# reczoo/FuxiCTR

Measured on NVIDIA H100. Metric: samples/sec DeepFM Criteo-shape train_step (fwd+bwd+clip+Adam), higher is better.
Workload: dtype f32 (3xTF32 tensor-core GEMMs, fp32 everything else)

## Files before the change

fuxictr_b200/_lib.py:

```python
import ctypes
import os

HERE = os.path.dirname(os.path.abspath(__file__))
LIB_PATH = os.path.join(HERE, "libfuxictr_b200.so")

B2_F32, B2_BF16, B2_F64, B2_I64, B2_I32 = 0, 1, 2, 3, 4
B2_POOL_NONE, B2_POOL_SUM, B2_POOL_MEAN = 0, 1, 2
B2_ACT_NONE, B2_ACT_RELU, B2_ACT_SIGMOID = 0, 1, 2
B2_PREP_MUL = 3
B2_GEMM_C_IS_ZERO, B2_GEMM_COLSUM_IS_ZERO, B2_GEMM_X3_INLINE, B2_GEMM_BACKFILL = 1, 2, 4, 8
B2_MAX_FIELDS = 128
FM_PRODUCT_SUM, FM_BI_INTERACTION, FM_INNER_PRODUCT = 0, 1, 2

c_void_p, c_int, c_int32, c_int64, c_float = (ctypes.c_void_p, ctypes.c_int, ctypes.c_int32,
                                              ctypes.c_int64, ctypes.c_float)


class b2_lazy_ctx(ctypes.Structure):
    _fields_ = [
        ("last_step", ctypes.c_void_p), ("sched", ctypes.c_void_p), ("step_dev", ctypes.c_void_p),
        ("mark", ctypes.c_void_p), ("worklist", ctypes.c_void_p), ("counter", ctypes.c_void_p),
        ("delta_m", ctypes.c_int64), ("delta_v", ctypes.c_int64),
        ("w1", ctypes.c_float), ("beta2", ctypes.c_float), ("w2", ctypes.c_float), ("eps", ctypes.c_float),
        ("worklist_capacity", ctypes.c_int32), ("pad_", ctypes.c_int32),
        ("grow_emb", ctypes.c_int64 * 128), ("grow_lr", ctypes.c_int64 * 128),
    ]


class b2_lazy_table(ctypes.Structure):
    _fields_ = [("param", ctypes.c_void_p), ("rows", ctypes.c_int64), ("grow_base", ctypes.c_int64),
                ("dim", ctypes.c_int32), ("pad_", ctypes.c_int32)]


class b2_field(ctypes.Structure):
    _fields_ = [
        ("table", c_void_p), ("idx", c_void_p), ("out", c_void_p),
        ("vocab", c_int64), ("idx_stride", c_int64), ("out_stride", c_int64),
        ("dim", c_int32), ("seq_len", c_int32), ("pool", c_int32), ("padding_idx", c_int32),
    ]


class b2_touch(ctypes.Structure):
    _fields_ = [("flags", c_void_p), ("base", c_void_p), ("n", c_int64)]


_FIELD_P = ctypes.POINTER(b2_field)


class b2_gemm_desc(ctypes.Structure):
    _fields_ = [
        ("a", c_void_p), ("b", c_void_p), ("a_small", c_void_p), ("b_small", c_void_p),
        ("c", c_void_p), ("c_small", c_void_p), ("c_pre", c_void_p), ("bias", c_void_p), ("mul", c_void_p), ("add", c_void_p),
        ("ybwd", c_void_p), ("colsum", c_void_p),
        ("lda", c_int64), ("ldb", c_int64), ("ldc", c_int64), ("M", c_int64), ("N", c_int64), ("K", c_int64),
        ("a_mn_major", c_int32), ("b_mn_major", c_int32), ("act", c_int32), ("act_bwd", c_int32),
        ("beta_accumulate", c_int32), ("elem_dtype", c_int32), ("ld_aux", c_int64),
        ("flags", c_int64),
        ("drop_rng", c_void_p), ("drop_layer", c_int64), ("drop_thresh", ctypes.c_uint32), ("drop_scale", c_float),
    ]

class b2_gemm_plan(ctypes.Structure):
    _fields_ = [(k, c_int32) for k in ("bn", "splits", "stages", "cstages", "grid", "threads", "tiles_m", "tiles_n",
                                       "passes", "kb_per_split")] + \
               [("smem_bytes", c_int64)]


SIGNATURES = {
    "b2_version": (ctypes.c_char_p, []),
    "b2_last_error": (ctypes.c_char_p, []),
    "b2_device_cc": (c_int, [c_int]),
    "b2_set_l2_fetch_granularity": (c_int, [c_int]),
    "b2_embed_gather_fwd": (c_int, [_FIELD_P, c_int, c_int64, c_int, c_int, c_void_p, c_void_p, c_void_p]),
    "b2_embed_gather_hot_fwd": (c_int, [_FIELD_P, c_int, c_int64, c_int, c_int, c_void_p, c_void_p, c_int, c_void_p]),
    "b2_embed_scatter_bwd": (c_int, [_FIELD_P, c_int, c_int64, c_int, c_int, c_void_p, c_void_p]),
    "b2_embed_scatter_bwd_ex": (c_int, [_FIELD_P, c_int, c_int64, c_int, c_int, c_void_p, c_void_p, c_void_p]),
    "b2_lr_fwd": (c_int, [_FIELD_P, c_int, c_int64, c_int, c_void_p, c_void_p, c_void_p, c_void_p]),
    "b2_lr_bwd": (c_int, [_FIELD_P, c_int, c_int64, c_int, c_void_p, c_void_p, c_void_p]),
    "b2_lr_bwd_ex": (c_int, [_FIELD_P, c_int, c_int64, c_int, c_void_p, c_void_p, c_void_p, c_void_p]),
    "b2_front_fwd": (c_int, [_FIELD_P, _FIELD_P, c_int, c_int64, c_int, c_int, c_void_p, c_void_p, c_void_p,
                             c_void_p, c_void_p, c_void_p, c_void_p]),
    "b2_front_bwd": (c_int, [_FIELD_P, _FIELD_P, c_int, c_int64, c_int, c_int, c_void_p, c_void_p, c_void_p,
                             c_void_p, c_void_p, c_void_p, c_void_p]),
    "b2_front_bwd_ex": (c_int, [_FIELD_P, _FIELD_P, c_int, c_int64, c_int, c_int, c_void_p, c_void_p, c_void_p,
                                c_void_p, c_void_p, c_void_p, c_void_p, c_void_p]),
    "b2_lazy_sumsq": (c_int, [c_void_p, c_int, c_void_p, c_void_p, c_int, c_int64, c_void_p, c_void_p]),
    "b2_lazy_adam_step": (c_int, [c_void_p, c_int, c_void_p, c_void_p, c_int, c_int64, c_int64, c_int64, c_void_p,
                                  c_void_p, c_void_p, c_void_p, c_float, c_float, c_float, c_float, c_void_p]),
    "b2_lazy_materialize": (c_int, [c_void_p, c_int, c_int64, c_int64, c_int64, c_void_p, c_void_p, c_void_p,
                                    c_float, c_float, c_float, c_void_p]),
    "b2_adam_sched": (c_int, [c_void_p, c_float, c_float, c_float, c_void_p, c_int64, c_void_p]),
    "b2_adam_step_sched": (c_int, [c_void_p, c_void_p, c_void_p, c_void_p, c_int64, c_void_p, c_float, c_float,
                                   c_float, c_float, c_void_p, c_void_p, c_int, c_void_p]),
    "b2_shard_push": (c_int, [_FIELD_P, _FIELD_P, c_int, c_int64, c_int, c_int, c_void_p, c_int, c_int64,
                              c_void_p, c_void_p, c_void_p, c_void_p, c_void_p, c_int32, c_void_p]),
    "b2_shard_pull": (c_int, [_FIELD_P, _FIELD_P, c_int, c_int64, c_int, c_int, c_void_p, c_void_p, c_float,
                              c_void_p, c_void_p, c_int32, c_void_p]),
    "b2_shard_push_ex": (c_int, [_FIELD_P, _FIELD_P, c_int, c_int64, c_int, c_int, c_void_p, c_int, c_int64,
                                 c_void_p, c_void_p, c_void_p, c_void_p, c_void_p, c_int32, c_void_p, c_void_p]),
    "b2_shard_pull_ex": (c_int, [_FIELD_P, _FIELD_P, c_int, c_int64, c_int, c_int, c_void_p, c_void_p, c_float,
                                 c_void_p, c_void_p, c_int32, c_void_p, c_void_p, c_void_p]),
    "b2_shard_push_pad": (c_int, [_FIELD_P, _FIELD_P, c_int, c_int64, c_int, c_int, c_void_p, c_int, c_int64,
                                  c_void_p, c_void_p, c_void_p, c_void_p, c_void_p, c_int32, c_void_p, c_void_p,
                                  c_void_p]),
    "b2_shard_publish_ids": (c_int, [c_void_p, c_int, c_int64, c_void_p, _FIELD_P, _FIELD_P, c_int, c_int, c_int,
                                     c_void_p, c_void_p]),
    "b2_shard_publish_rows": (c_int, [c_void_p, c_int, c_int64, c_int64, c_int64, c_void_p, _FIELD_P, _FIELD_P, c_int,
                                      c_int, c_int, c_void_p, c_void_p, c_void_p]),
    "b2_shard_lookup": (c_int, [_FIELD_P, _FIELD_P, c_int, c_int64, c_int, c_int, c_void_p, c_int64, c_void_p, c_void_p,
                                c_void_p, c_void_p, c_void_p, c_void_p]),
    "b2_peer_bcast": (c_int, [c_void_p, c_int64, c_void_p, c_int, c_void_p]),
    "b2_peer_bcast_ids": (c_int, [c_void_p, c_int, c_int64, c_void_p, c_int, c_void_p]),
# ... 106 lines not shown
```

fuxictr_b200/csrc/gemm_tc.cu:

```cuda
#include "b2_common.cuh"
#include "philox.cuh"
#include <string.h>
#include <cstdlib>
#include <cuda.h>

namespace tc {
constexpr int BM = 128;
constexpr int NTHREADS = 384;
constexpr int NCONV = 96;
constexpr int BACKFILL_KB = 16;
enum Mode { TF32 = 0, BF16 = 1, X3 = 2 };

struct Ring {
  uint32_t off_b, off_as, off_bs, off_sa, off_sb;
  uint32_t stage;
  int stages;
  size_t smem;
};
constexpr uint32_t RING_EXTRA = 1024 + 128;
constexpr uint32_t SMEM_MAX = 227u * 1024u;
constexpr Ring ring_layout(int bn, int mode, bool a_mn, bool b_mn) {
  const uint32_t a = BM * 128, b = (uint32_t) bn * 128;
  Ring r{};
  uint32_t o = a;
// ... 5 lines not shown
  r.stage = o;
  r.stages = (SMEM_MAX - RING_EXTRA) / o >= 4 ? 4 : (int) ((SMEM_MAX - RING_EXTRA) / o);
  r.smem = (size_t) r.stages * o + RING_EXTRA;
  return r;
}
constexpr size_t ring_smem_max(int bn, int mode) {
  size_t m = 0;
  for (int a_mn = 0; a_mn < 2; ++a_mn)
    for (int b_mn = 0; b_mn < 2; ++b_mn) {
      const size_t s = ring_layout(bn, mode, a_mn != 0, b_mn != 0).smem;
      m = s > m ? s : m;
    }
  return m;
}
static_assert(ring_layout(128, TF32, true, true).stages >= 2 && ring_layout(64, X3, true, true).stages >= 2,
              "ring does not fit shared memory");
constexpr int epi_pitch(int bn) { return bn + 8; }
constexpr uint32_t epi_bytes(int bn) { return (uint32_t) (BM * epi_pitch(bn) + 256 * 4) * 4u; }
constexpr bool epi_fits(int bn, int mode) {
  for (int a_mn = 0; a_mn < 2; ++a_mn)
    for (int b_mn = 0; b_mn < 2; ++b_mn) {
      const Ring r = ring_layout(bn, mode, a_mn != 0, b_mn != 0);
      if ((uint32_t) r.stages * r.stage < epi_bytes(bn)) return false;
    }
  return true;
}
static_assert(epi_fits(32, TF32) && epi_fits(64, TF32) && epi_fits(128, TF32) && epi_fits(32, BF16) &&
              epi_fits(64, BF16) && epi_fits(128, BF16) && epi_fits(32, X3) && epi_fits(64, X3),
              "epilogue tile does not fit the ring");

struct Params {
  CUtensorMap map_a;
  CUtensorMap map_b;
  float* c;
  float* c_small;
  float* c_pre;
  int64_t ldc;
  const float* bias;
  const float* mul;
  const float* add;
  const float* ybwd;
  float* colsum;
  int M, N, K, act, act_bwd, beta, kb_per_split;
  int a_mn, b_mn;
  int esz;
  int64_t ld_aux;
  int vec;
  int tiles_m, tiles_n, splits;
  Ring ring;
  const int64_t* drop_rng;
  int64_t drop_layer;
  uint32_t drop_thresh;
  float drop_scale;
};

__device__ __forceinline__ uint32_t smem_u32(const void* p) {
  return (uint32_t) __cvta_generic_to_shared(p);
}
__device__ __forceinline__ void mbar_init(uint32_t bar, uint32_t count) {
  asm volatile("mbarrier.init.shared::cta.b64 [%0], %1;" ::"r"(bar), "r"(count) : "memory");
}
__device__ __forceinline__ void mbar_expect_tx(uint32_t bar, uint32_t bytes) {
  asm volatile("mbarrier.arrive.expect_tx.shared::cta.b64 _, [%0], %1;" ::"r"(bar), "r"(bytes)
               : "memory");
}
__device__ __forceinline__ void mbar_arrive(uint32_t bar) {
  asm volatile("mbarrier.arrive.shared::cta.b64 _, [%0];" ::"r"(bar) : "memory");
}
__device__ __forceinline__ bool mbar_try_wait(uint32_t bar, uint32_t parity) {
  uint32_t ok;
  asm volatile(
      "{\n"
      ".reg .pred p;\n"
      "mbarrier.try_wait.parity.shared::cta.b64 p, [%1], %2;\n"
      "selp.u32 %0, 1, 0, p;\n"
      "}\n"
      : "=r"(ok)
      : "r"(bar), "r"(parity)
      : "memory");
  return ok != 0;
}
__device__ __forceinline__ void mbar_wait(uint32_t bar, uint32_t parity) {
  if (mbar_try_wait(bar, parity)) return;
  const long long t0 = clock64();
  while (!mbar_try_wait(bar, parity))
    if (clock64() - t0 > 4000000000LL) __trap();
}
__device__ __forceinline__ void tma_load_2d(uint32_t dst, const CUtensorMap* map, uint32_t bar,
                                            int c0, int c1) {
  asm volatile(
      "cp.async.bulk.tensor.2d.shared::cluster.global.mbarrier::complete_tx::bytes [%0], [%1, {%2, %3}], [%4];"
      ::"r"(dst), "l"(reinterpret_cast<uint64_t>(map)), "r"(c0), "r"(c1), "r"(bar)
      : "memory");
}
__device__ __forceinline__ uint64_t make_smem_desc(uint32_t addr) {
  uint64_t d = 0;
  d |= (uint64_t) ((addr & 0x3FFFFu) >> 4);
  d |= (uint64_t) 1 << 16;
  d |= (uint64_t) (1024 >> 4) << 32;
  d |= (uint64_t) 1 << 62;
  return d;
}
__device__ __forceinline__ uint32_t swz(int r, int c) { return (uint32_t) (r * 128 + ((c ^ (r & 7)) << 4)); }
__device__ __forceinline__ float tf32_small(float v) { return b2_tf32_small(v); }
__device__ __forceinline__ float tf32_big(float v) { return __uint_as_float(__float_as_uint(v) & 0xffffe000u); }
__device__ __forceinline__ void wgmma_fence() { asm volatile("wgmma.fence.sync.aligned;" ::: "memory"); }
// ... 361 lines not shown
    constexpr int SEG = BM * SPR / 256;
    constexpr int BATCH = 4;
    const int et = threadIdx.x - 128;
    const int c4 = et % SPR, r0 = et / SPR;
    const int n = n0 + 4 * c4;
    const int nv = min(4, p.N - n);
    const bool vec_n = p.vec && nv == 4;
    const float4 bv = (p.bias != nullptr && z == 0 && nv > 0) ? seg_load<true>(p.bias + n, vec_n, nv)
                                                             : make_float4(0.f, 0.f, 0.f, 0.f);
    float cs[4] = {0.f, 0.f, 0.f, 0.f};
    uint64_t dseed = 0, doff = 0;
    if constexpr (DROP) {
      dseed = (uint64_t) p.drop_rng[0];
      doff = (uint64_t) p.drop_rng[1] + (uint64_t) p.drop_layer;
    }
#pragma unroll 1
    for (int b0 = 0; b0 < SEG; b0 += BATCH) {
      float4 mv[BATCH], av[BATCH], yv[BATCH], cv[BATCH];
#pragma unroll
      for (int i = 0; i < BATCH; ++i) {
        const int m = m0 + r0 + (256 / SPR) * (b0 + i);
        const int k = m < p.M ? nv : 0;
        const bool v = vec_n && m < p.M;
        const int64_t o = (int64_t) m * p.ldc + n;
        const float4 zero = make_float4(0.f, 0.f, 0.f, 0.f);
        mv[i] = p.mul != nullptr ? seg_load<true>(p.mul + o, v, k) : zero;
        av[i] = p.add != nullptr ? seg_load<true>(p.add + o, v, k) : zero;
        yv[i] = p.ybwd != nullptr ? seg_load<true>(p.ybwd + o, v, k) : zero;
        cv[i] = (p.beta && p.splits == 1) ? seg_load<false>(p.c + o, v, k) : zero;
      }
#pragma unroll
      for (int i = 0; i < BATCH; ++i) {
        const int r = r0 + (256 / SPR) * (b0 + i);
        const int m = m0 + r;
        const int k = m < p.M ? nv : 0;
        const bool v = vec_n && m < p.M;
        const int64_t o = (int64_t) m * p.ldc + n;
        const float4 a = *reinterpret_cast<const float4*>(tile + r * P + 4 * c4);
        float4 t = make_float4(__fadd_rn(a.x, bv.x), __fadd_rn(a.y, bv.y), __fadd_rn(a.z, bv.z), __fadd_rn(a.w, bv.w));
        if (p.splits > 1) {
          seg_red_add(p.c + o, t, v, k);
          continue;
        }
        if (p.c_pre != nullptr) seg_store(p.c_pre + o, t, v, k);
        uint32_t kb = 0;
        if constexpr (DROP) {
          if (k > 0) kb = b2_drop_keep4(dseed, doff, (uint64_t) m * (uint64_t) p.N + (uint64_t) n, k, p.drop_thresh);
        }
        t.x = epilogue_elem<DROP>(p, t.x, mv[i].x, av[i].x, yv[i].x, cv[i].x, kb & 1u);
        t.y = epilogue_elem<DROP>(p, t.y, mv[i].y, av[i].y, yv[i].y, cv[i].y, kb & 2u);
        t.z = epilogue_elem<DROP>(p, t.z, mv[i].z, av[i].z, yv[i].z, cv[i].z, kb & 4u);
        t.w = epilogue_elem<DROP>(p, t.w, mv[i].w, av[i].w, yv[i].w, cv[i].w, kb & 8u);
        seg_store(p.c + o, t, v, k);
        if (p.c_small != nullptr) {
          const int64_t oa = (int64_t) m * p.ld_aux + n;
          if (p.esz == 4)
            seg_store(p.c_small + oa, make_float4(tf32_small(t.x), tf32_small(t.y), tf32_small(t.z), tf32_small(t.w)), v, k);
          else
            seg_store_bf16(reinterpret_cast<__nv_bfloat16*>(p.c_small) + oa, t, v, k);
        }
        if (k > 0) cs[0] += t.x;
        if (k > 1) cs[1] += t.y;
        if (k > 2) cs[2] += t.z;
        if (k > 3) cs[3] += t.w;
      }
    }
    if (p.colsum != nullptr) {
      float* part = tile + BM * P;
      *reinterpret_cast<float4*>(part + 4 * et) = make_float4(cs[0], cs[1], cs[2], cs[3]);
      consumer_sync();
      if (et < BN && n0 + et < p.N) {
        float s = 0.f;
#pragma unroll
        for (int u = et >> 2; u < 256; u += SPR) s += part[4 * u + (et & 3)];
        b2_red_add(p.colsum + n0 + et, s);
      }
    }
  }
}

__global__ void __launch_bounds__(256)
split_tf32_kernel(const float* __restrict__ x, float* __restrict__ small, int64_t n) {
  b2_pdl_wait();
  b2_pdl_trigger();
  for (int64_t i = (int64_t) blockIdx.x * blockDim.x + threadIdx.x; i < n;
       i += (int64_t) gridDim.x * blockDim.x) {
    small[i] = tf32_small(x[i]);
  }
}

__global__ void __launch_bounds__(256)
transpose_kernel(const float* __restrict__ in, int64_t rows, int64_t cols, int64_t ld_in,
                 float* __restrict__ out, int64_t ld_out, float* __restrict__ out_small) {
  __shared__ float tile[32][33];
  const int tx = threadIdx.x & 31, ty = threadIdx.x >> 5;
  const int64_t c0 = (int64_t) blockIdx.x * 32, r0 = (int64_t) blockIdx.y * 32;
#pragma unroll
  for (int i = 0; i < 32; i += 8) {
    const int64_t r = r0 + ty + i, c = c0 + tx;
    tile[ty + i][tx] = (r < rows && c < cols) ? __ldg(in + r * ld_in + c) : 0.f;
  }
  __syncthreads();
#pragma unroll
  for (int i = 0; i < 32; i += 8) {
    const int64_t c = c0 + ty + i, r = r0 + tx;
    if (c < cols && r < rows) {
      const float v = tile[tx][ty + i];
      out[c * ld_out + r] = v;
      if (out_small != nullptr)
        out_small[c * ld_out + r] = tf32_small(v);
    }
  }
}

template <bool DROP>
__global__ void __launch_bounds__(256)
prep_operand_kernel(const float* __restrict__ x, const float* __restrict__ y, int act, int64_t R,
                    int64_t C, int64_t ld_in, float* __restrict__ out, float* __restrict__ out_small,
                    float* __restrict__ outT, float* __restrict__ outT_small, float* __restrict__ colsum,
                    const int64_t* __restrict__ drop_rng, int64_t drop_layer, uint32_t drop_thresh, float drop_scale) {
  b2_pdl_wait();
  b2_pdl_trigger();
  __shared__ float tile[32][33];
  const int tx = threadIdx.x & 31, ty = threadIdx.x >> 5;
// ... 229 lines not shown
}

template <int BN, int MODE, bool DROP>
static int gemm_launch(const tc::Params& p, int grid, cudaStream_t st) {
  void (*kern)(tc::Params) = tc::gemm_tc_kernel<BN, MODE, DROP>;
  static const cudaError_t attr_rc =
      cudaFuncSetAttribute(kern, cudaFuncAttributeMaxDynamicSharedMemorySize, (int) tc::ring_smem_max(BN, MODE));
  if (attr_rc != cudaSuccess) return b2_fail(B2_E_CUDA, "b2_gemm_tc: smem attribute: %s", cudaGetErrorString(attr_rc));
  B2_REQUIRE(p.ring.smem <= tc::ring_smem_max(BN, MODE), "ring exceeds the shared-memory attribute");
  B2_LAUNCH(kern, grid, tc::NTHREADS, p.ring.smem, st, p);
  B2_CUDA_LAUNCH_CHECK("b2_gemm_tc");
  return B2_OK;
}

typedef int (*GemmLaunch)(const tc::Params&, int, cudaStream_t);
template <bool DROP>
static GemmLaunch gemm_inst_t(int bn, int mode) {
  switch (bn * 4 + mode) {
    case 32 * 4 + tc::TF32: return gemm_launch<32, tc::TF32, DROP>;
    case 64 * 4 + tc::TF32: return gemm_launch<64, tc::TF32, DROP>;
    case 128 * 4 + tc::TF32: return gemm_launch<128, tc::TF32, DROP>;
    case 32 * 4 + tc::BF16: return gemm_launch<32, tc::BF16, DROP>;
    case 64 * 4 + tc::BF16: return gemm_launch<64, tc::BF16, DROP>;
    case 128 * 4 + tc::BF16: return gemm_launch<128, tc::BF16, DROP>;
    case 32 * 4 + tc::X3: return gemm_launch<32, tc::X3, DROP>;
    case 64 * 4 + tc::X3: return gemm_launch<64, tc::X3, DROP>;
    default: return nullptr;
  }
}
static GemmLaunch gemm_inst(int bn, int mode, bool drop) {
  return drop ? gemm_inst_t<true>(bn, mode) : gemm_inst_t<false>(bn, mode);
}

static int gemm_tc_impl(const b2_gemm_desc* d, void* stream, b2_gemm_plan* plan) {
  B2_REQUIRE(d != nullptr, "NULL descriptor");
  const void* a = d->a; const void* b = d->b; float* c = d->c;
  const int64_t M = d->M, N = d->N, K = d->K, lda = d->lda, ldb = d->ldb, ldc = d->ldc;
  B2_REQUIRE(a && b && c, "NULL operand");
  B2_REQUIRE(d->elem_dtype == B2_F32 || d->elem_dtype == B2_BF16, "operand dtype must be B2_F32 or B2_BF16");
  const int esz = (d->elem_dtype == B2_BF16) ? 2 : 4;
  B2_REQUIRE(M >= 1 && N >= 1 && K >= 1 && ldc >= N, "bad shape");
  B2_REQUIRE(M < (1ll << 31) && N < (1ll << 31) && K < (1ll << 31), "shape exceeds 31 bits");
  B2_REQUIRE(lda >= (d->a_mn_major ? M : K) && ldb >= (d->b_mn_major ? N : K), "leading dimension too small");
  B2_REQUIRE(d->act >= B2_ACT_NONE && d->act <= B2_ACT_SIGMOID, "bad activation code %d", d->act);
  B2_REQUIRE(d->act_bwd >= B2_ACT_NONE && d->act_bwd <= B2_ACT_SIGMOID, "bad act_bwd code %d", d->act_bwd);
  B2_REQUIRE(d->act_bwd == B2_ACT_NONE || d->ybwd != nullptr, "act_bwd needs ybwd");
  B2_REQUIRE((d->a_small == nullptr) == (d->b_small == nullptr), "3xTF32 needs both small operands");
  B2_REQUIRE(esz == 4 || d->a_small == nullptr, "bf16 operands are single-pass (no small parts)");
  const bool inline_split = (d->flags & B2_GEMM_X3_INLINE) != 0;
  B2_REQUIRE(!inline_split || (esz == 4 && d->a_small == nullptr), "B2_GEMM_X3_INLINE: fp32 operands, no small parts");
  const bool three_pass = inline_split || d->a_small != nullptr;
  const int64_t ld_aux = d->ld_aux > 0 ? d->ld_aux : ldc;
  B2_REQUIRE(d->c_small == nullptr || ld_aux >= N, "ld_aux too small");
  const bool drop = d->drop_rng != nullptr;
  B2_REQUIRE(!drop || (d->drop_scale > 0.f && d->drop_scale < 3.0e38f && d->drop_layer >= 0),
             "dropout needs a positive finite scale and a layer index >= 0");
  if (!tma_ok_e(a, lda, esz) || !tma_ok_e(b, ldb, esz) ||
      (d->a_small != nullptr && !(tma_ok(d->a_small, lda) && tma_ok(d->b_small, ldb))))
    return b2_fail(B2_E_UNSUPPORTED, "operands are not TMA-addressable (16-byte base, 16-byte row pitch)");
  cudaStream_t st = (cudaStream_t) stream;

  const int bke = 128 / esz;
  const int64_t tiles_m = b2_ceil_div(M, tc::BM);
  const int64_t num_kb = b2_ceil_div(K, bke);
  const bool linear = (d->act == B2_ACT_NONE && d->mul == nullptr && d->add == nullptr && d->ybwd == nullptr &&
                       d->c_small == nullptr && d->c_pre == nullptr && d->colsum == nullptr && !drop);
  const bool backfill = (d->flags & B2_GEMM_BACKFILL) != 0;
  int best_bn = 0, best_split = 1;
  double best_cost = 1e300;
  const int bn_max = three_pass ? 64 : 128;
  for (int bn = 32; bn <= bn_max; bn *= 2) {
    const bool mn_a = d->a_mn_major != 0, mn_b = d->b_mn_major != 0;
    const double passes = three_pass ? 3.0 : 1.0;
    const double rows_tma = tc::BM + bn;
    const double rows_conv = (mn_a ? 2.0 : 0.0) * tc::BM + (mn_b ? 2.0 : 0.0) * bn +
                             (three_pass ? (mn_a ? 1.0 : 0.0) * tc::BM + (mn_b ? 1.0 : 2.0) * bn : 0.0);
    const double rows_mma = passes * 2.0 * bn + (three_pass && !mn_a ? 1.0 : passes) * tc::BM;
    const double per_kb = fmax(passes * 4.0 * bn, rows_tma + rows_conv + rows_mma);
    const int64_t tiles_n = b2_ceil_div(N, bn);
    for (int split = 1; split <= 32; split *= 2) {
      if (split > 1 && (!linear || num_kb / split < 8)) break;
      const int64_t ctas = tiles_m * tiles_n * split;
      const int64_t waves = b2_ceil_div(ctas, B2_NUM_SMS);
      const double kb = (double) b2_ceil_div(num_kb, split);
      const double cost = (double) waves * (10000.0 + kb * per_kb);
      if (cost < best_cost) { best_cost = cost; best_bn = bn; best_split = split; }
    }
  }
  if (backfill && linear) {
    while (best_split < 32 && num_kb / (2 * best_split) >= tc::BACKFILL_KB) best_split *= 2;
  }
  tc::Params p;
  memset(&p, 0, sizeof(p));
  if (plan == nullptr) {
    int rc = encode_operand(&p.map_a, a, M, K, lda, d->a_mn_major, tc::BM, esz);
    if (rc != B2_OK) return rc;
    rc = encode_operand(&p.map_b, b, N, K, ldb, d->b_mn_major, best_bn, esz);
    if (rc != B2_OK) return rc;
  }
  p.c = c; p.c_small = reinterpret_cast<float*>(d->c_small); p.c_pre = d->c_pre; p.ldc = ldc; p.ld_aux = ld_aux;
  p.bias = d->bias; p.mul = d->mul; p.add = d->add;
  p.ybwd = d->ybwd; p.colsum = d->colsum;
  p.M = (int) M; p.N = (int) N; p.K = (int) K; p.act = d->act; p.act_bwd = d->act_bwd; p.esz = esz;
  p.a_mn = d->a_mn_major ? 1 : 0; p.b_mn = d->b_mn_major ? 1 : 0;
  p.beta = d->beta_accumulate ? 1 : 0;
  p.drop_rng = d->drop_rng; p.drop_layer = d->drop_layer; p.drop_thresh = d->drop_thresh; p.drop_scale = d->drop_scale;
  {
    auto al = [](const void* q, uintptr_t b) { return reinterpret_cast<uintptr_t>(q) % b == 0; };
    p.vec = al(c, 16) && ldc % 4 == 0 && al(d->c_pre, 16) && al(d->bias, 16) && al(d->mul, 16) &&
            al(d->add, 16) && al(d->ybwd, 16) && al(d->c_small, esz == 4 ? 16 : 8) &&
            (d->c_small == nullptr || ld_aux % 4 == 0);
  }
  p.kb_per_split = (int) b2_ceil_div(num_kb, best_split);
  const int splits = (int) b2_ceil_div(num_kb, p.kb_per_split);
  const int64_t tiles_n = b2_ceil_div(N, best_bn);
  const int64_t total_tiles = tiles_m * tiles_n * splits;
  B2_REQUIRE(total_tiles < (1ll << 31), "too many tiles");
  p.tiles_m = (int) tiles_m; p.tiles_n = (int) tiles_n; p.splits = splits;
  const int mode = three_pass ? tc::X3 : (esz == 2 ? tc::BF16 : tc::TF32);
  const GemmLaunch launch = gemm_inst(best_bn, mode, drop);
  B2_REQUIRE(launch != nullptr, "no GEMM instantiation for bn %d", best_bn);
  p.ring = tc::ring_layout(best_bn, mode, p.a_mn != 0, p.b_mn != 0);
  B2_REQUIRE(p.ring.stages >= 2 && p.ring.smem <= tc::SMEM_MAX, "tile does not fit shared memory");
  if (plan != nullptr) {
    plan->bn = best_bn; plan->splits = splits; plan->stages = p.ring.stages; plan->cstages = p.ring.stages;
    plan->grid = (int) total_tiles; plan->threads = tc::NTHREADS; plan->tiles_m = p.tiles_m; plan->tiles_n = p.tiles_n;
    plan->passes = three_pass ? 3 : 1; plan->kb_per_split = p.kb_per_split; plan->smem_bytes = (int64_t) p.ring.smem;
    return B2_OK;
  }
  if (splits > 1 && !p.beta && !(d->flags & B2_GEMM_C_IS_ZERO)) {
    cudaError_t e = cudaMemset2DAsync(c, (size_t) ldc * 4, 0, (size_t) N * 4, (size_t) M, st);
    if (e != cudaSuccess) return b2_fail(B2_E_CUDA, "b2_gemm_tc: memset: %s", cudaGetErrorString(e));
  }
  if (d->colsum != nullptr && !(d->flags & B2_GEMM_COLSUM_IS_ZERO)) {
    cudaError_t e = cudaMemsetAsync(d->colsum, 0, sizeof(float) * (size_t) N, st);
    if (e != cudaSuccess) return b2_fail(B2_E_CUDA, "b2_gemm_tc: memset: %s", cudaGetErrorString(e));
  }
  return launch(p, (int) total_tiles, st);
}

extern "C" B2_API int b2_gemm_tc_ex(const b2_gemm_desc* d, void* stream) { return gemm_tc_impl(d, stream, nullptr); }

extern "C" B2_API int b2_gemm_tc_plan(const b2_gemm_desc* d, b2_gemm_plan* plan) {
  B2_REQUIRE(plan != nullptr, "NULL plan");
  return gemm_tc_impl(d, nullptr, plan);
}

namespace tc {
__global__ void __launch_bounds__(256)
to_bf16_kernel(const float* __restrict__ x, int64_t rows, int64_t cols, int64_t ld_in,
               __nv_bfloat16* __restrict__ out, int64_t ld_out) {
  const int64_t n = rows * cols;
  for (int64_t i = (int64_t) blockIdx.x * blockDim.x + threadIdx.x; i < n; i += (int64_t) gridDim.x * blockDim.x) {
    const int64_t r = i / cols, c = i - r * cols;
    out[r * ld_out + c] = __float2bfloat16_rn(__ldg(x + r * ld_in + c));
  }
}
}

// ... 163 lines not shown
```

fuxictr_b200/functional.py:

```python
import ctypes
import os
import weakref

import torch

from . import _lib
from ._lib import (B2_F32, B2_BF16, B2_F64, B2_I32, B2_I64, B2_POOL_NONE, B2_POOL_SUM, B2_POOL_MEAN,
                   B2_ACT_NONE, B2_ACT_RELU, B2_ACT_SIGMOID, B2_PREP_MUL, b2_field)

_IDX_CODE = {torch.float64: B2_F64, torch.int64: B2_I64, torch.int32: B2_I32}
ACT_CODE = {None: B2_ACT_NONE, "none": B2_ACT_NONE, "relu": B2_ACT_RELU, "sigmoid": B2_ACT_SIGMOID}


def _stream():
    return ctypes.c_void_p(torch.cuda.current_stream().cuda_stream)


def _ptr(t):
    return ctypes.c_void_p(t.data_ptr()) if t is not None else ctypes.c_void_p(0)


def _require_cuda(*tensors):
    for t in tensors:
        if t is not None and not t.is_cuda:
# ... 302 lines not shown
        b_rs, b_cs = b.stride(1), b.stride(0)
    else:
        K2, N = b.shape
        b_rs, b_cs = b.stride(0), b.stride(1)
    if K != K2 or tuple(out.shape) != (M, N) or out.stride(1) != 1:
        raise ValueError("gemm shape mismatch: a%s b%s out%s" % (tuple(a.shape), tuple(b.shape), tuple(out.shape)))
    _lib.call("b2_gemm_f32", _ptr(a), a_rs, a_cs, _ptr(b), b_rs, b_cs, _ptr(out), out.stride(0), M, N, K,
              _ptr(bias), act, _ptr(mul), _ptr(add), 1 if accumulate else 0, _stream())
    return out


_MATMUL = {"mode": "fp32", "x3_inline": os.environ.get("B2_X3_INLINE", "1") != "0"}


def set_x3_inline(on):
    _MATMUL["x3_inline"] = bool(on)


def _x3_aux():
    return _MATMUL["mode"] == "tf32x3" and not _MATMUL["x3_inline"]


def set_matmul_precision(mode):
    if mode not in ("fp32", "tf32x3", "tf32", "bf16"):
        raise ValueError("matmul precision must be 'fp32', 'tf32x3', 'tf32' or 'bf16'")
    _MATMUL["mode"] = mode


def get_matmul_precision():
    return _MATMUL["mode"]


def _tc_operand_ok(t):
    return t.dim() == 2 and t.stride(1) == 1 and t.stride(0) % 4 == 0 and t.data_ptr() % 16 == 0 \
        and t.stride(0) >= t.shape[1]


def split_tf32(t):
    small = torch.empty_like(t)
    _lib.call("b2_split_tf32", _ptr(t), _ptr(small), t.numel(), _stream())
    return small


def transpose_f32(t, want_small):
    rows, cols = t.shape
    out = torch.empty((cols, rows), dtype=torch.float32, device=t.device)
    small = torch.empty_like(out) if want_small else None
    _lib.call("b2_transpose_f32", _ptr(t), rows, cols, t.stride(0), _ptr(out), rows, _ptr(small), _stream())
    return out, small


def gemm_ex(a, b, out, a_mn=False, b_mn=False, a_small=None, b_small=None, bias=None, act=B2_ACT_NONE,
            mul=None, add=None, ybwd=None, act_bwd=B2_ACT_NONE, out_small=None, colsum=None, accumulate=False,
            out_pre=None, out_is_zero=False, backfill=False, drop=None):
    d = _lib.b2_gemm_desc()
    K, M = (a.shape if a_mn else a.shape[::-1])
    K2, N = (b.shape if b_mn else b.shape[::-1])
    if K != K2 or tuple(out.shape) != (M, N) or out.stride(1) != 1 or a.stride(1) != 1 or b.stride(1) != 1:
        raise ValueError("gemm_ex shape mismatch: a%s b%s out%s" % (tuple(a.shape), tuple(b.shape), tuple(out.shape)))
    for t in (mul, add, ybwd, out_pre) + ((out_small,) if (out_small is not None and out_small.dtype == torch.float32) else ()):
        if t is not None and (tuple(t.shape) != (M, N) or t.stride(0) != out.stride(0) or t.stride(1) != 1):
            raise ValueError("gemm_ex: epilogue tensors must share out's shape and leading dimension")
    bf16 = a_small is not None and a_small.dtype == torch.bfloat16
    if bf16:
        if b_small is None or b_small.dtype != torch.bfloat16 or a_small.shape != a.shape or b_small.shape != b.shape:
            raise ValueError("gemm_ex: bf16 mode needs bf16 copies of both operands")
        a, b, a_small, b_small = a_small, b_small, None, None
        d.elem_dtype = B2_BF16
    for t, ref in ((a_small, a), (b_small, b)):
        if t is not None and (t.shape != ref.shape or t.stride() != ref.stride()):
            raise ValueError("gemm_ex: small parts must share their operand's layout")
    d.a, d.b = a.data_ptr(), b.data_ptr()
    d.a_small = a_small.data_ptr() if a_small is not None else None
    d.b_small = b_small.data_ptr() if b_small is not None else None
    d.c = out.data_ptr()
    d.c_small = out_small.data_ptr() if out_small is not None else None
    if out_small is not None:
        if (out_small.dtype == torch.bfloat16) != bf16:
            raise ValueError("gemm_ex: out_small dtype does not match the operand mode")
        d.ld_aux = out_small.stride(0)
    d.c_pre = out_pre.data_ptr() if out_pre is not None else None
    d.bias = bias.data_ptr() if bias is not None else None
    d.mul = mul.data_ptr() if mul is not None else None
    d.add = add.data_ptr() if add is not None else None
    d.ybwd = ybwd.data_ptr() if ybwd is not None else None
    d.colsum = colsum.data_ptr() if colsum is not None else None
    d.lda, d.ldb, d.ldc = a.stride(0), b.stride(0), out.stride(0)
    d.M, d.N, d.K = M, N, K
    d.a_mn_major, d.b_mn_major = int(bool(a_mn)), int(bool(b_mn))
    d.act, d.act_bwd = act, (act_bwd if ybwd is not None else B2_ACT_NONE)
    d.beta_accumulate = 1 if accumulate else 0
    d.flags = (_lib.B2_GEMM_C_IS_ZERO if out_is_zero else 0) | (_lib.B2_GEMM_COLSUM_IS_ZERO if _is_zeroed(colsum) else 0) \
        | (_lib.B2_GEMM_BACKFILL if backfill else 0)
    if a_small is None and not bf16 and _MATMUL["mode"] == "tf32x3" and _MATMUL["x3_inline"]:
        d.flags |= _lib.B2_GEMM_X3_INLINE
    if drop is not None:
        d.drop_rng, d.drop_layer, d.drop_thresh, d.drop_scale = drop[0].data_ptr(), drop[1], drop[2], drop[3]
    _lib.call("b2_gemm_tc_ex", ctypes.byref(d), _stream())
    return out


def gemm_nt(a, b, out, bias=None, act=B2_ACT_NONE, mul=None, add=None, accumulate=False,
            a_small=None, b_small=None):
    mode = _MATMUL["mode"]
    N = b.shape[0]
    use_tc = (mode != "fp32" and N >= 16 and _tc_operand_ok(a) and _tc_operand_ok(b) and out.stride(1) == 1)
    if not use_tc:
        return gemm_f32(a, b, out, b_t=True, bias=bias, act=act, mul=mul, add=add, accumulate=accumulate)
    if mode in ("tf32x3", "bf16"):
        if a_small is None:
            a_small = make_aux(a)
        if b_small is None:
            b_small = make_aux(b)
    else:
        a_small = b_small = None
    return gemm_ex(a, b, out, a_small=a_small, b_small=b_small, bias=bias, act=act, mul=mul, add=add,
                   accumulate=accumulate)


_WEIGHT_EPOCH = [0]
_SMALL_CACHE = {}


def bump_weight_epoch():
    _WEIGHT_EPOCH[0] += 1


def _pad8(n):
    return (n + 7) // 8 * 8


def empty_aux(rows, cols, device):
    mode = _MATMUL["mode"]
    if _x3_aux():
# ... 158 lines not shown
        gb = _grad_buffer(ctx.bias, zero=False) if need_b else None
        fused = act != B2_ACT_NONE
        if ctx.kind == "tc":
            x3 = _x3_aux()
            gz, gz_small, _, _ = prep_operand(gy, y if fused else None, act, want_out=fused, want_small=x3, colsum=gb)
            if not fused:
                gz = gy
            if not x3:
                gz_small = make_aux(gz)
            if need_x:
                gx = torch.empty((M, K), dtype=torch.float32, device=x.device)
                gemm_ex(gz, weight, gx, b_mn=True, a_small=gz_small, b_small=weight_aux(weight))
            if need_w:
                gw = _grad_buffer(weight, zero=False)
                gemm_ex(gz, x, gw, a_mn=True, b_mn=True, a_small=gz_small, b_small=ctx.x_small,
                        out_is_zero=_is_zeroed(gw))
            return gx, gw, gb, None
        gz = gy
        if fused or gb is not None:
            out, _, _, _ = prep_operand(gy, y if fused else None, act, want_out=fused, colsum=gb)
            if fused:
                gz = out
        if need_x:
            gx = torch.empty((M, K), dtype=torch.float32, device=x.device)
            gemm_f32(gz, weight, gx)
        if need_w:
            gw = _grad_buffer(weight, zero=False)
            gemm_f32(gz, x, gw, a_t=True)
        return gx, gw, gb, None


_FORK = {"on": True, "side": {}}


def set_backward_fork(on):
    _FORK["on"] = bool(on)


class _WgradFork(object):

    def __init__(self, dev):
        side = _FORK["side"].get(dev)
        if side is None:
            side = _FORK["side"][dev] = torch.cuda.Stream(device=dev)
        self.main, self.side = torch.cuda.current_stream(dev), side
        self.keep, self.arenas = [], set()
        self.defer = True

    def ready(self):
        ev = torch.cuda.Event()
        ev.record(self.main)
        return ev

    def gemm(self, ready, gz, gz_small, h, h_small, gw):
        self.side.wait_event(ready)
        with torch.cuda.stream(self.side):
            gemm_ex(gz, h, gw, a_mn=True, b_mn=True, a_small=gz_small, b_small=h_small,
                    out_is_zero=_is_zeroed(gw), backfill=True)
        self.keep += [gz, gz_small, h, h_small]
        base = gw._base
        arena = getattr(base, "_b2_arena", None) if base is not None else None
        if arena is None or not arena.defer_join:
            self.defer = False
        else:
            self.arenas.add(arena)

    def join(self):
        done = torch.cuda.Event()
        done.record(self.side)
        if self.defer and len(self.arenas) == 1:
            self.arenas.pop().pending.append((done, self.keep))
        else:
            self.main.wait_event(done)


class _MLPChain(torch.autograd.Function):

    @staticmethod
    def forward(ctx, x, acts, drops, *params):
        x = _f32c(x)
        M = x.shape[0]
        L = len(acts)
        Ws, bs = params[0::2], params[1::2]
        x3 = _x3_aux()
        dl = [None] * L
        n_drop = sum(1 for p in (drops or ()) if p > 0)
        snap = dropout_snapshot(x.device, n_drop) if n_drop else None
        for i, p in enumerate(drops or ()):
            if p > 0:
                dl[i] = (snap, sum(1 for q in drops[:i] if q > 0)) + dropout_consts(p)
        kinds = []
        for W in Ws:
            if W.shape[0] == 1 and W.is_contiguous():
                kinds.append("head")
            elif _tc_layer_ok(W):
                kinds.append("tc")
            else:
                kinds.append("simt")
        hs = [x]
        smalls = [make_aux(x) if kinds[0] == "tc" else None]
        for i in range(L):
            W, b, act = Ws[i], bs[i], acts[i]
            N, K = W.shape
            h = hs[-1]
            y = torch.empty((M, N), dtype=torch.float32, device=x.device)
            want_small = i + 1 < L and kinds[i + 1] == "tc"
            y_small = None
            if kinds[i] == "head":
                _lib.call("b2_head_fwd", _ptr(h), _ptr(W), _ptr(b), M, K, act, _ptr(y), _stream())
            elif kinds[i] == "tc" and h.data_ptr() % 16 == 0:
                y_small = empty_aux(M, N, x.device) if want_small else None
                gemm_ex(h, W, y, a_small=smalls[-1], b_small=weight_aux(W), bias=b, act=act, out_small=y_small,
                        drop=dl[i])
            else:
                kinds[i] = "simt"
                gemm_f32(h, W, y, b_t=True, bias=b, act=act)
            if dl[i] is not None and kinds[i] != "tc":
                dropout_apply(y, snap, dl[i][1], drops[i], out=y)
            if want_small and y_small is None:
                y_small = make_aux(y)
            hs.append(y)
            smalls.append(y_small)
        ctx.acts, ctx.kinds, ctx.smalls, ctx.params, ctx.dl = acts, kinds, smalls, params, dl
        ctx.save_for_backward(*hs)
        return hs[-1]

    @staticmethod
    def backward(ctx, gy):
        hs = ctx.saved_tensors
        acts, kinds, smalls, params, dl = ctx.acts, ctx.kinds, ctx.smalls, ctx.params, ctx.dl
        Ws, bs = params[0::2], params[1::2]
        L = len(acts)
        M = hs[0].shape[0]
        dev = hs[0].device
        x3 = _x3_aux()
        grads = [None] * len(params)

        def bias_buf(i):
            b = bs[i]
            return _grad_buffer(b, zero=False) if (b is not None and b.requires_grad) else None

        g, g_small, g_is_dz = _f32c(gy), None, False
        fork = None
        for i in range(L - 1, -1, -1):
            W, act, h, y = Ws[i], acts[i], hs[i], hs[i + 1]
            N, K = W.shape
            need_gx = i > 0 or ctx.needs_input_grad[0]
            fuse_prev = i > 0
            prev_small = fuse_prev and kinds[i - 1] == "tc"
            gx = torch.empty((M, K), dtype=torch.float32, device=dev) if need_gx else None
            gx_small = empty_aux(M, K, dev) if (prev_small and gx is not None) else None
            gb_prev = None
            if kinds[i] == "head":
                if dl[i] is not None and not g_is_dz:
                    gb = bias_buf(i)
                    g, _, _, _ = prep_operand(g, y if act != B2_ACT_NONE else None, act, want_out=True, colsum=gb,
                                              drop=dl[i])
                    grads[2 * i + 1] = gb
                    g_is_dz = True
                gw = _grad_buffer(W, zero=False)
                gb = None if g_is_dz else bias_buf(i)
                gb_prev = bias_buf(i - 1) if fuse_prev else None
                fp32_small = gx_small if (gx_small is not None and gx_small.dtype == torch.float32) else None
                pdrop = dl[i - 1] if fuse_prev else None
                _lib.call("b2_head_bwd_ex", _ptr(h), _ptr(W), None if g_is_dz else _ptr(y), _ptr(g), M, K,
                          B2_ACT_NONE if g_is_dz else act, _ptr(gx), _ptr(gw), _ptr(gb),
                          acts[i - 1] if fuse_prev else B2_ACT_NONE, _ptr(fp32_small), _ptr(gb_prev),
                          1 if (_is_zeroed(gw) and (gb is None or _is_zeroed(gb))
                                and (gb_prev is None or _is_zeroed(gb_prev))) else 0,
                          *((_ptr(pdrop[0]),) + pdrop[1:] if pdrop is not None else (_ptr(None), 0, 0, 0.0)),
                          _stream())
                if gx_small is not None and fp32_small is None:
                    gx_small = make_aux(gx)
                grads[2 * i] = gw
                if not g_is_dz:
                    grads[2 * i + 1] = gb
                if fuse_prev:
                    grads[2 * (i - 1) + 1] = gb_prev
                g, g_small, g_is_dz = gx, gx_small, fuse_prev
                continue
            if not g_is_dz:
                gb = bias_buf(i)
                fused = act != B2_ACT_NONE
                out, sm, _, _ = prep_operand(g, y if fused else None, act, want_out=fused or dl[i] is not None,
                                             want_small=x3 and kinds[i] == "tc", colsum=gb, drop=dl[i])
                gz, gz_small = (out if (fused or dl[i] is not None) else g), sm
                if gz_small is None and kinds[i] == "tc":
                    gz_small = make_aux(gz)
                grads[2 * i + 1] = gb
            else:
                gz, gz_small = g, g_small
            if kinds[i] == "tc":
                if fork is None and W.requires_grad and _FORK["on"] and gz.is_cuda:
                    fork = _WgradFork(dev)
                ready = fork.ready() if (fork is not None and W.requires_grad) else None
                if gx is not None:
                    prev_act = acts[i - 1] if fuse_prev else B2_ACT_NONE
                    gb_prev = bias_buf(i - 1) if fuse_prev else None
                    gemm_ex(gz, W, gx, b_mn=True, a_small=gz_small, b_small=weight_aux(W),
                            ybwd=hs[i] if (fuse_prev and prev_act != B2_ACT_NONE) else None, act_bwd=prev_act,
                            out_small=gx_small, colsum=gb_prev,
                            drop=dl[i - 1] if fuse_prev else None)
                if W.requires_grad:
                    gw = _grad_buffer(W, zero=False)
                    if ready is not None:
                        fork.gemm(ready, gz, gz_small, h, smalls[i], gw)
                    else:
                        gemm_ex(gz, h, gw, a_mn=True, b_mn=True, a_small=gz_small, b_small=smalls[i],
                                out_is_zero=_is_zeroed(gw))
                    grads[2 * i] = gw
                g, g_small, g_is_dz = gx, gx_small, fuse_prev
            else:
                if gx is not None:
                    gemm_f32(gz, W, gx)
                if W.requires_grad:
                    gw = _grad_buffer(W, zero=False)
                    gemm_f32(gz, h, gw, a_t=True)
                    grads[2 * i] = gw
                g, g_small, g_is_dz = gx, None, False
                continue
            if fuse_prev:
                grads[2 * (i - 1) + 1] = gb_prev
        if fork is not None:
            fork.join()
        return (g if ctx.needs_input_grad[0] else None, None, None) + tuple(grads)


class _CrossV2Layer(torch.autograd.Function):

    @staticmethod
    def forward(ctx, x0, xi, weight, bias):
        x0, xi = _f32c(x0), _f32c(xi)
        M, d = xi.shape
        out = torch.empty_like(xi)
        lin = torch.empty_like(xi)
        ctx.tc = (_tc_layer_ok(weight) and weight.shape[0] == weight.shape[1] == d
                  and xi.data_ptr() % 16 == 0 and x0.data_ptr() % 16 == 0)
        ctx.xi_small = None
        if ctx.tc:
            ctx.xi_small = make_aux(xi)
            gemm_ex(xi, weight, out, a_small=ctx.xi_small, b_small=weight_aux(weight), bias=bias,
                    mul=x0, add=xi, out_pre=lin)
        else:
            gemm_f32(xi, weight, lin, b_t=True, bias=bias)
            torch.addcmul(xi, x0, lin, out=out)
        ctx.save_for_backward(x0, xi, lin, weight)
        ctx.bias = bias
        return out

    @staticmethod
    def backward(ctx, g):
        x0, xi, lin, weight = ctx.saved_tensors
        g = _f32c(g)
        bias = ctx.bias
        gb = _grad_buffer(bias, zero=False) if (bias is not None and bias.requires_grad) else None
        x3 = _x3_aux()
        dlin, dlin_small, _, _ = prep_operand(g, x0, B2_PREP_MUL, want_out=True, want_small=x3 and ctx.tc, colsum=gb)
        if ctx.tc and dlin_small is None:
            dlin_small = make_aux(dlin)
        gxi = torch.empty_like(xi)
        gw = _grad_buffer(weight, zero=False) if weight.requires_grad else None
        if ctx.tc:
            gemm_ex(dlin, weight, gxi, b_mn=True, a_small=dlin_small, b_small=weight_aux(weight),
                    add=g)
            if gw is not None:
                gemm_ex(dlin, xi, gw, a_mn=True, b_mn=True, a_small=dlin_small, b_small=ctx.xi_small, out_is_zero=_is_zeroed(gw))
        else:
            gemm_f32(dlin, weight, gxi, add=g)
            if gw is not None:
                gemm_f32(dlin, xi, gw, a_t=True)
        gx0 = g * lin if ctx.needs_input_grad[0] else None
        return gx0, gxi, gw, gb
# ... 373 lines not shown
```

include/fuxictr_b200.h:

```cpp
#ifndef FUXICTR_B200_H_
#define FUXICTR_B200_H_

#include <stdint.h>

#if defined(__GNUC__)
#define B2_API __attribute__((visibility("default")))
#else
#define B2_API
#endif

#ifdef __cplusplus
extern "C" {
#endif

#define B2_OK 0
#define B2_E_INVALID (-1)
#define B2_E_CUDA (-2)
#define B2_E_UNSUPPORTED (-3)

#define B2_F32 0
#define B2_BF16 1
#define B2_F64 2
#define B2_I64 3
#define B2_I32 4
// ... 166 lines not shown
                       double* stats_ws, float* out, void* stream);
B2_API int b2_dice_bwd(const float* x, const float* gout, const float* alpha, const float* mean,
                       const float* rstd, int64_t M, int C, int training, double* stats_ws, float* gx,
                       float* galpha, void* stream);
B2_API int b2_din_input_fwd(const float* target, const float* hist, int64_t B, int L, int d, float* out,
                            void* stream);
B2_API int b2_din_input_bwd(const float* target, const float* hist, const float* gin, int64_t B, int L, int d,
                            float* gtarget, float* ghist, int accumulate_hist, void* stream);
B2_API int b2_din_wsum_fwd(const float* w, const unsigned char* mask, const float* hist, int64_t B, int L,
                           int d, float* out, void* stream);
B2_API int b2_din_wsum_bwd(const float* w, const unsigned char* mask, const float* hist, const float* gout,
                           int64_t B, int L, int d, float* gw, float* ghist, void* stream);
B2_API int b2_din_softmax_fwd(const float* w, const unsigned char* mask, int64_t B, int L, float* p, void* stream);
B2_API int b2_din_softmax_bwd(const float* p, const float* g, const unsigned char* mask, int64_t B, int L,
                              float* gw, void* stream);

B2_API int b2_gemm_f32(const float* a, int64_t a_rs, int64_t a_cs, const float* b, int64_t b_rs,
                int64_t b_cs, float* c, int64_t ldc, int64_t M, int64_t N, int64_t K,
                const float* bias, int act, const float* mul, const float* add,
                int beta_accumulate, void* stream);

B2_API int b2_gemm_tc_supported(const float* a, int64_t lda, const float* b, int64_t ldb, int64_t M,
                                int64_t N, int64_t K);
B2_API int b2_gemm_tc(const float* a, int64_t lda, const float* b, int64_t ldb, float* c, int64_t ldc,
                      int64_t M, int64_t N, int64_t K, const float* bias, int act, const float* mul,
                      const float* add, int beta_accumulate, const float* a_small,
                      const float* b_small, void* stream);

typedef struct b2_gemm_desc {
  const void* a;
  const void* b;
  const float* a_small;
  const float* b_small;
  float* c;
  void* c_small;
  float* c_pre;
  const float* bias;
  const float* mul;
  const float* add;
  const float* ybwd;
  float* colsum;
  int64_t lda, ldb, ldc;
  int64_t M, N, K;
  int32_t a_mn_major, b_mn_major;
  int32_t act, act_bwd;
  int32_t beta_accumulate;
  int32_t elem_dtype;
  int64_t ld_aux;
  int64_t flags;
  const int64_t* drop_rng;
  int64_t drop_layer;
  uint32_t drop_thresh;
  float drop_scale;
} b2_gemm_desc;
#define B2_GEMM_C_IS_ZERO 1
#define B2_GEMM_COLSUM_IS_ZERO 2
#define B2_GEMM_X3_INLINE 4
#define B2_GEMM_BACKFILL 8
B2_API int b2_gemm_tc_ex(const b2_gemm_desc* desc, void* stream);
typedef struct b2_gemm_plan {
  int32_t bn, splits, stages, cstages, grid, threads, tiles_m, tiles_n, passes, kb_per_split;
  int64_t smem_bytes;
} b2_gemm_plan;
B2_API int b2_gemm_tc_plan(const b2_gemm_desc* desc, b2_gemm_plan* plan);
B2_API int b2_to_bf16(const float* x, int64_t rows, int64_t cols, int64_t ld_in, void* out, int64_t ld_out,
                      void* stream);
B2_API int b2_split_tf32(const float* x, float* small, int64_t n, void* stream);
B2_API int b2_transpose_f32(const float* in, int64_t rows, int64_t cols, int64_t ld_in, float* out,
                            int64_t ld_out, float* out_small, void* stream);

B2_API int b2_prep_operand(const float* x, const float* y, int act, int64_t R, int64_t C, float* out,
                           float* out_small, float* outT, float* outT_small, float* colsum,
                           const int64_t* drop_rng, int64_t drop_layer, uint32_t drop_thresh, float drop_scale,
                           void* stream);
B2_API int b2_head_fwd(const float* x, const float* w, const float* b, int64_t M, int K, int act, float* y,
                       void* stream);
B2_API int b2_head_bwd(const float* x, const float* w, const float* y, const float* gy, int64_t M, int K,
                       int act, float* gx, float* gw, float* gb, void* stream);
B2_API int b2_head_bwd_ex(const float* x, const float* w, const float* y, const float* gy, int64_t M, int K,
                          int act, float* gx, float* gw, float* gb, int prev_act, float* gx_small,
                          float* gb_prev, int grads_zeroed, const int64_t* prev_drop_rng, int64_t prev_drop_layer,
                          uint32_t prev_drop_thresh, float prev_drop_scale, void* stream);

B2_API int b2_dropout_rng_take(int64_t* state, int64_t* snapshot, int n_layers, void* stream);
B2_API int b2_dropout_apply(const float* x, float* y, int64_t M, int64_t N, int64_t ld, const int64_t* snapshot,
                            int64_t layer, uint32_t thresh, float scale, void* stream);
B2_API int b2_act_bwd(const float* y, const float* gy, float* gx, int64_t n, int act, void* stream);
B2_API int b2_colsum(const float* x, int64_t M, int64_t N, int64_t ld, float* out, int accumulate,
              void* stream);

B2_API int b2_logit_bce_fwd(const float* t0, const float* t1, const float* t2, const float* t3,
                     const float* label, int64_t batch, float* y_pred, float* loss,
                     float* glogit, void* stream);

B2_API int b2_sumsq(const float* g, int64_t n, float* out, void* stream);
B2_API int b2_adam_step(float* p, float* g, float* m, float* v, int64_t n, const float* sumsq,
                 float max_norm, float lr, float beta1, float beta2, float eps,
                 const int64_t* step_dev, int zero_grad, void* stream);
B2_API int b2_sumsq_ex(const float* g, int64_t n, float* out, const uint8_t* flags, int64_t n_flagged,
                       void* stream);
B2_API int b2_adam_step_ex(float* p, float* g, float* m, float* v, int64_t n, const float* sumsq,
                           float max_norm, float lr, float beta1, float beta2, float eps,
                           const int64_t* step_dev, int zero_grad, uint8_t* flags, int64_t n_flagged,
                           void* stream);
B2_API int b2_adam_untouched(float* p, float* m, float* v, int64_t n, const uint8_t* flags, float lr, float beta1,
                             float beta2, float eps, const int64_t* step_dev, int max_ctas, void* stream);
// ... 20 lines not shown
```

Measured before the change: 8.545 million.

## Emit transposed gradient from dgrad GEMM epilogue for K-major weight-grad GEMMs

```diff
diff --git a/fuxictr_b200/_lib.py b/fuxictr_b200/_lib.py
--- a/fuxictr_b200/_lib.py
+++ b/fuxictr_b200/_lib.py
@@ -57,6 +57,7 @@
         ("beta_accumulate", c_int32), ("elem_dtype", c_int32), ("ld_aux", c_int64),
         ("flags", c_int64),
         ("drop_rng", c_void_p), ("drop_layer", c_int64), ("drop_thresh", ctypes.c_uint32), ("drop_scale", c_float),
+        ("c_t", c_void_p), ("ld_t", c_int64),
     ]
 
 class b2_gemm_plan(ctypes.Structure):
diff --git a/fuxictr_b200/csrc/gemm_tc.cu b/fuxictr_b200/csrc/gemm_tc.cu
--- a/fuxictr_b200/csrc/gemm_tc.cu
+++ b/fuxictr_b200/csrc/gemm_tc.cu
@@ -81,6 +81,9 @@
   int64_t drop_layer;
   uint32_t drop_thresh;
   float drop_scale;
+  float* c_t;
+  int64_t ld_t;
+  int vec_t;
 };
 
 __device__ __forceinline__ uint32_t smem_u32(const void* p) {
@@ -548,6 +551,7 @@
         t.z = epilogue_elem<DROP>(p, t.z, mv[i].z, av[i].z, yv[i].z, cv[i].z, kb & 4u);
         t.w = epilogue_elem<DROP>(p, t.w, mv[i].w, av[i].w, yv[i].w, cv[i].w, kb & 8u);
         seg_store(p.c + o, t, v, k);
+        if (p.c_t != nullptr) *reinterpret_cast<float4*>(tile + r * P + 4 * c4) = t;
         if (p.c_small != nullptr) {
           const int64_t oa = (int64_t) m * p.ld_aux + n;
           if (p.esz == 4)
@@ -561,11 +565,30 @@
         if (k > 3) cs[3] += t.w;
       }
     }
-    if (p.colsum != nullptr) {
+    if (p.c_t != nullptr || p.colsum != nullptr) {
       float* part = tile + BM * P;
-      *reinterpret_cast<float4*>(part + 4 * et) = make_float4(cs[0], cs[1], cs[2], cs[3]);
+      if (p.colsum != nullptr) *reinterpret_cast<float4*>(part + 4 * et) = make_float4(cs[0], cs[1], cs[2], cs[3]);
       consumer_sync();
-      if (et < BN && n0 + et < p.N) {
+      if (p.c_t != nullptr) {
+        const int qq = lane & 3, cc = lane >> 2;
+#pragma unroll 4
+        for (int j = 0; j < BN / 8; ++j) {
+          const int u = (et >> 5) + 8 * j;
+          const int r = 4 * (4 * (u & 7) + qq), c = 8 * (u >> 3) + cc;
+          const int m = m0 + r, n = n0 + c;
+          if (m >= p.M || n >= p.N) continue;
+          float x[4];
+#pragma unroll
+          for (int i = 0; i < 4; ++i) x[i] = tile[(r + ((i + qq) & 3)) * P + c];
+          auto row = [&](int j) {
+            const int i = (j - qq) & 3;
+            return i == 0 ? x[0] : i == 1 ? x[1] : i == 2 ? x[2] : x[3];
+          };
+          const int mv = min(4, p.M - m);
+          seg_store(p.c_t + (int64_t) n * p.ld_t + m, make_float4(row(0), row(1), row(2), row(3)), p.vec_t && mv == 4, mv);
+        }
+      }
+      if (p.colsum != nullptr && et < BN && n0 + et < p.N) {
         float s = 0.f;
 #pragma unroll
         for (int u = et >> 2; u < 256; u += SPR) s += part[4 * u + (et & 3)];
@@ -901,6 +924,7 @@
   const bool three_pass = inline_split || d->a_small != nullptr;
   const int64_t ld_aux = d->ld_aux > 0 ? d->ld_aux : ldc;
   B2_REQUIRE(d->c_small == nullptr || ld_aux >= N, "ld_aux too small");
+  B2_REQUIRE(d->c_t == nullptr || d->ld_t >= M, "ld_t too small");
   const bool drop = d->drop_rng != nullptr;
   B2_REQUIRE(!drop || (d->drop_scale > 0.f && d->drop_scale < 3.0e38f && d->drop_layer >= 0),
              "dropout needs a positive finite scale and a layer index >= 0");
@@ -913,7 +937,8 @@
   const int64_t tiles_m = b2_ceil_div(M, tc::BM);
   const int64_t num_kb = b2_ceil_div(K, bke);
   const bool linear = (d->act == B2_ACT_NONE && d->mul == nullptr && d->add == nullptr && d->ybwd == nullptr &&
-                       d->c_small == nullptr && d->c_pre == nullptr && d->colsum == nullptr && !drop);
+                       d->c_small == nullptr && d->c_pre == nullptr && d->colsum == nullptr && d->c_t == nullptr &&
+                       !drop);
   const bool backfill = (d->flags & B2_GEMM_BACKFILL) != 0;
   int best_bn = 0, best_split = 1;
   double best_cost = 1e300;
@@ -954,6 +979,8 @@
   p.a_mn = d->a_mn_major ? 1 : 0; p.b_mn = d->b_mn_major ? 1 : 0;
   p.beta = d->beta_accumulate ? 1 : 0;
   p.drop_rng = d->drop_rng; p.drop_layer = d->drop_layer; p.drop_thresh = d->drop_thresh; p.drop_scale = d->drop_scale;
+  p.c_t = d->c_t; p.ld_t = d->ld_t;
+  p.vec_t = reinterpret_cast<uintptr_t>(d->c_t) % 16 == 0 && d->ld_t % 4 == 0;
   {
     auto al = [](const void* q, uintptr_t b) { return reinterpret_cast<uintptr_t>(q) % b == 0; };
     p.vec = al(c, 16) && ldc % 4 == 0 && al(d->c_pre, 16) && al(d->bias, 16) && al(d->mul, 16) &&
diff --git a/fuxictr_b200/functional.py b/fuxictr_b200/functional.py
--- a/fuxictr_b200/functional.py
+++ b/fuxictr_b200/functional.py
@@ -378,7 +378,7 @@
 
 def gemm_ex(a, b, out, a_mn=False, b_mn=False, a_small=None, b_small=None, bias=None, act=B2_ACT_NONE,
             mul=None, add=None, ybwd=None, act_bwd=B2_ACT_NONE, out_small=None, colsum=None, accumulate=False,
-            out_pre=None, out_is_zero=False, backfill=False, drop=None):
+            out_pre=None, out_is_zero=False, backfill=False, drop=None, out_t=None):
     d = _lib.b2_gemm_desc()
     K, M = (a.shape if a_mn else a.shape[::-1])
     K2, N = (b.shape if b_mn else b.shape[::-1])
@@ -406,6 +406,10 @@
             raise ValueError("gemm_ex: out_small dtype does not match the operand mode")
         d.ld_aux = out_small.stride(0)
     d.c_pre = out_pre.data_ptr() if out_pre is not None else None
+    if out_t is not None:
+        if tuple(out_t.shape) != (N, M) or out_t.stride(1) != 1 or out_t.dtype != torch.float32:
+            raise ValueError("gemm_ex: out_t must be fp32 (N, M) with unit column stride")
+        d.c_t, d.ld_t = out_t.data_ptr(), out_t.stride(0)
     d.bias = bias.data_ptr() if bias is not None else None
     d.mul = mul.data_ptr() if mul is not None else None
     d.add = add.data_ptr() if add is not None else None
@@ -670,10 +674,10 @@
         ev.record(self.main)
         return ev
 
-    def gemm(self, ready, gz, gz_small, h, h_small, gw):
+    def gemm(self, ready, gz, gz_small, h, h_small, gw, a_mn=True, b_mn=True):
         self.side.wait_event(ready)
         with torch.cuda.stream(self.side):
-            gemm_ex(gz, h, gw, a_mn=True, b_mn=True, a_small=gz_small, b_small=h_small,
+            gemm_ex(gz, h, gw, a_mn=a_mn, b_mn=b_mn, a_small=gz_small, b_small=h_small,
                     out_is_zero=_is_zeroed(gw), backfill=True)
         self.keep += [gz, gz_small, h, h_small]
         base = gw._base
@@ -690,6 +694,14 @@
             self.arenas.pop().pending.append((done, self.keep))
         else:
             self.main.wait_event(done)
+
+
+def _kmajor_wgrads(x):
+    return _FORK["on"] and x.is_cuda and _MATMUL["mode"] == "tf32x3" and not _x3_aux()
+
+
+def _t_buffer(rows, M, dev):
+    return torch.empty((rows, (M + 3) // 4 * 4), dtype=torch.float32, device=dev)[:, :M]
 
 
 class _MLPChain(torch.autograd.Function):
@@ -759,6 +771,8 @@
             return _grad_buffer(b, zero=False) if (b is not None and b.requires_grad) else None
 
         g, g_small, g_is_dz = _f32c(gy), None, False
+        g_t = None
+        wt = _kmajor_wgrads(hs[0])
         fork = None
         for i in range(L - 1, -1, -1):
             W, act, h, y = Ws[i], acts[i], hs[i], hs[i + 1]
@@ -768,6 +782,7 @@
             prev_small = fuse_prev and kinds[i - 1] == "tc"
             gx = torch.empty((M, K), dtype=torch.float32, device=dev) if need_gx else None
             gx_small = empty_aux(M, K, dev) if (prev_small and gx is not None) else None
+            gx_t = None
             gb_prev = None
             if kinds[i] == "head":
                 if dl[i] is not None and not g_is_dz:
@@ -815,19 +830,23 @@
                 if gx is not None:
                     prev_act = acts[i - 1] if fuse_prev else B2_ACT_NONE
                     gb_prev = bias_buf(i - 1) if fuse_prev else None
+                    if wt and prev_small and Ws[i - 1].requires_grad:
+                        gx_t = _t_buffer(K, M, dev)
                     gemm_ex(gz, W, gx, b_mn=True, a_small=gz_small, b_small=weight_aux(W),
                             ybwd=hs[i] if (fuse_prev and prev_act != B2_ACT_NONE) else None, act_bwd=prev_act,
                             out_small=gx_small, colsum=gb_prev,
-                            drop=dl[i - 1] if fuse_prev else None)
+                            drop=dl[i - 1] if fuse_prev else None, out_t=gx_t)
                 if W.requires_grad:
                     gw = _grad_buffer(W, zero=False)
-                    if ready is not None:
+                    if ready is not None and g_t is not None:
+                        fork.gemm(ready, g_t, None, h, smalls[i], gw, a_mn=False)
+                    elif ready is not None:
                         fork.gemm(ready, gz, gz_small, h, smalls[i], gw)
                     else:
                         gemm_ex(gz, h, gw, a_mn=True, b_mn=True, a_small=gz_small, b_small=smalls[i],
                                 out_is_zero=_is_zeroed(gw))
                     grads[2 * i] = gw
-                g, g_small, g_is_dz = gx, gx_small, fuse_prev
+                g, g_small, g_is_dz, g_t = gx, gx_small, fuse_prev, gx_t
             else:
                 if gx is not None:
                     gemm_f32(gz, W, gx)
@@ -835,7 +854,7 @@
                     gw = _grad_buffer(W, zero=False)
                     gemm_f32(gz, h, gw, a_t=True)
                     grads[2 * i] = gw
-                g, g_small, g_is_dz = gx, None, False
+                g, g_small, g_is_dz, g_t = gx, None, False, None
                 continue
             if fuse_prev:
                 grads[2 * (i - 1) + 1] = gb_prev
diff --git a/include/fuxictr_b200.h b/include/fuxictr_b200.h
--- a/include/fuxictr_b200.h
+++ b/include/fuxictr_b200.h
@@ -242,6 +242,8 @@
   int64_t drop_layer;
   uint32_t drop_thresh;
   float drop_scale;
+  float* c_t;
+  int64_t ld_t;
 } b2_gemm_desc;
 #define B2_GEMM_C_IS_ZERO 1
 #define B2_GEMM_COLSUM_IS_ZERO 2
```

Result: faster. 8.706 million (median of 6 runs) (+1.9%).
